# sanowl/CUDA-NT-Xent-MPI-NCCL-SimCLR

Hardware: AMD Instinct MI355X
Metric: NT-Xent fwd+bwd samples/sec, B=4096 d=2048, at 1/2/4/8 MI355X (higher is better)
Workload: dtype bf16

## Files before the change

cuda-nt-xent-mpi-nccl-simclr_amd/csrc/include/ntxent/ntxent.h:

```cpp
#pragma once

#include <hip/hip_runtime.h>

#include <cstdint>
#include <stdexcept>
#include <string>
#include <vector>

namespace ntxent {

constexpr int kWaveSize = 64;
constexpr int kTile = 256;
constexpr int kTileElems = kTile * kTile;
constexpr int kKStepBytes = 128;
constexpr int kGemmThreads = 512;
constexpr int kLdsPerCU = 160 * 1024;
constexpr int kNumXcd = 8;

enum class DType : int { F32 = 0, F16 = 1, BF16 = 2, FP8 = 3 };

inline size_t dtype_size(DType t) { return t == DType::F32 ? 4 : (t == DType::FP8 ? 1 : 2); }
inline const char* dtype_name(DType t) {
  return t == DType::F32 ? "fp32" : (t == DType::F16 ? "fp16" : (t == DType::BF16 ? "bf16" : "fp8"));
}
// ... 120 lines not shown
int q8_ldt(const Geometry& g);
struct Q8Stats {
  float* mneg2 = nullptr;
  float* lmin = nullptr;
  void* zq8t = nullptr;
  const void* zq = nullptr;
};
void launch_lse(const float2* part, const float* ypos, float* lse2_all, float* cpos,
                float* block_loss, float* loss_sum, const Geometry& g, hipStream_t stream,
                DType tr_dtype = DType::F16, const void* zq = nullptr, void* zqt = nullptr,
                const Q8Stats* q8 = nullptr, const RawRows* raw = nullptr);

int dot_slots(const Geometry& g);
void launch_coef(DType comp, const void* sbuf, void* cbuf, const float* lse2_all, const float* cpos,
                 const int4* tiles, int ntiles, const Geometry& g, hipStream_t stream,
                 void* mbuf = nullptr, float* dotp = nullptr, const Q8Stats* q8 = nullptr, bool half_c = false);
void launch_dot_reduce(const float* dotp, float* dot, const Geometry& g, hipStream_t stream);

void launch_coef_gemm(DType comp, const void* zq_local, const void* zq_all, void* cbuf,
                      const float* lse2_all, const float* cpos, const int4* tiles, int ntiles,
                      const GemmWorkspace& ws, const Geometry& g, hipStream_t stream,
                      const BlockView& bv = BlockView{}, float* dotp = nullptr);

struct NormFuse {
  const void* h = nullptr;
  DType in = DType::BF16;
  const float* inv = nullptr;
  const float* dot = nullptr;
  const float* grad_out = nullptr;
  void* dh = nullptr;
  const float* dotp = nullptr;
  int* dot_cnt = nullptr;
};
bool launch_dz(DType comp, const void* cbuf, const void* zqt_all, const int4* tiles, int ntiles,
               void* dz, const GemmWorkspace& ws, const Geometry& g, hipStream_t stream, bool out_f16 = false,
               const NormFuse* nf = nullptr, const Q8Stats* q8 = nullptr, const float* cpos = nullptr,
               bool half_c = false);
bool dz_half_c_eligible(DType comp, const Geometry& g, int n_dz, const GemmWorkspace& ws);
void set_half_c(bool on);
bool half_c_enabled();
bool dz_dot_fold_eligible(DType comp, const Geometry& g, int n_dz, const GemmWorkspace& ws);
void set_dot_fold(bool on);
bool dot_fold_enabled();
void set_dot_fold_spin(int polls);
int dot_fold_spin();

void launch_dz_view(DType comp, const void* a, long long a_panel_tiles, const void* b, long long b_kblk_cols,
                    long long b_kblk_stride, int k_tiles, const int4* tiles, int ntiles, void* out, bool accum,
                    const GemmWorkspace& ws, const Geometry& g, hipStream_t stream, bool out_f16 = false);

void launch_norm_bwd(DType in, const float* slabs, int nslabs, const void* h,
                     const float* inv, const float* grad_out, void* dh, const Geometry& g,
                     hipStream_t stream, const void* xslabs = nullptr, int nx = 0);

constexpr int kSmallMaxRows = 2048;
// ... 29 lines not shown
```

cuda-nt-xent-mpi-nccl-simclr_amd/csrc/include/ntxent/step.h:

```cpp
#pragma once

#include <hip/hip_runtime.h>

#include <cstddef>

#include "ntxent/ntxent.h"

namespace ntxent {

struct StepOverrides {
  int small_path = -1;
  int small_splits = -1;
  int fp8_backward = -1;
};

struct StepPlan {
  Geometry g;
  DType in = DType::BF16;
  DType comp = DType::F16;
  DType bwd = DType::F16;
  bool keep_cos = true;
  bool small = false;
  bool small_fwd_fused = false;
  int small_splits = 0;
  bool f8 = false;
  bool q8 = false;
  bool raw = false;
  bool fuse = false;
  bool half_c = false;
  bool dfold = false;
  int n_fwd = 0, n_own = 0, n_dz = 0;
  int num_cus = 256;
  DType fwd_mfma = DType::F16;
  DType bwd_mfma = DType::F16;
};

StepPlan resolve_step_plan(const Geometry& g, DType in, DType comp, bool keep_cos, int num_cus,
                           const StepOverrides& ov = StepOverrides{});

struct StepBuffers {
  const void* h = nullptr;
  void* zq = nullptr;
  void* zq8 = nullptr;
  void* zqt = nullptr;
// ... 46 lines not shown
```

cuda-nt-xent-mpi-nccl-simclr_amd/csrc/kernels/ntxent_kernels.hip:

```cpp

#include "../include/ntxent/ntxent.h"
#include "device_common.h"
#include "sim_gemm.h"

#include <atomic>
#include <algorithm>
#include <cmath>
#include <cstdio>
#include <cstdlib>
#include <mutex>
#include <string>
#include <type_traits>
#include <vector>
#include <unordered_map>

namespace ntxent {
namespace dev {

template <typename T> __device__ __forceinline__ void load8(const T* p, float (&v)[8]);
template <> __device__ __forceinline__ void load8<float>(const float* p, float (&v)[8]) {
  const f32x4 a = *reinterpret_cast<const f32x4*>(p), b = *reinterpret_cast<const f32x4*>(p + 4);
  v[0] = a[0]; v[1] = a[1]; v[2] = a[2]; v[3] = a[3]; v[4] = b[0]; v[5] = b[1]; v[6] = b[2]; v[7] = b[3];
}
template <typename T> __device__ __forceinline__ void load8_h(const T* p, float (&v)[8]) {
// ... 743 lines not shown
      std::fclose(fp);
    }
  }
};
#endif

template <typename Tc, int MODE>
void launch_sim_gemm(int grid, const dev::SimParams& p_in, hipStream_t stream) {
#if NTXENT_TIMING
  static TimingBuf tb;
  dev::SimParams p = p_in;
  p.tstamp = tb.prepare(grid, stream);
#else
  const dev::SimParams& p = p_in;
#endif
  if (MODE == dev::kModeFwd && !p.fixed_shift)
    hipLaunchKernelGGL((dev::sim_gemm_kernel<Tc, MODE, MODE == dev::kModeFwd ? 0 : 1>), dim3(grid), dim3(kGemmThreads), 0,
                       stream, p);
  else
    hipLaunchKernelGGL((dev::sim_gemm_kernel<Tc, MODE>), dim3(grid), dim3(kGemmThreads), 0, stream, p);
#if NTXENT_TIMING
  tb.dump("gemm_m" + std::to_string(MODE) + "_e" + std::to_string(sizeof(Tc)), grid, stream);
#endif
}

dev::SimParams base_params(const Geometry& g) {
  dev::SimParams p{};
  p.R = g.rows;
  p.Rpad = g.rows_pad;
  p.n_half = g.rows / 2;
// ... 341 lines not shown
static std::atomic<bool> g_lse_fold{[] {
  const char* e = std::getenv("NTXENT_LSE_FOLD");
  return e == nullptr || std::string(e) != "0";
}()};
void set_lse_fold(bool on) { g_lse_fold = on; }

bool lse_fold_enabled() { return g_lse_fold.load(); }
static double lse_loss_fx(const Geometry& g, int nb);

static std::atomic<bool> g_half_c{[] {
  const char* e = std::getenv("NTXENT_HALF_C");
  return e == nullptr || std::string(e) != "0";
}()};
void set_half_c(bool on) { g_half_c = on; }
bool half_c_enabled() { return g_half_c.load(); }

bool dz_half_c_eligible(DType comp, const Geometry& g, int n_dz, const GemmWorkspace& ws) {
  if ((comp != DType::F16 && comp != DType::BF16) || g.world != 1 || n_dz <= 0) return false;
  if ((long long)g.row_tiles * g.col_tiles * kTileElems * 2 >= (1ll << 31)) return false;
  const int cus = ws.sched_cus > 0 ? std::min(ws.sched_cus, ws.num_cus) : ws.num_cus;
  const int nk = (int)((long long)g.rows_pad * 2 / kKStepBytes);
  int pieces = fwd_splitk_pieces(n_dz, nk, cus, 1);
  if (pieces < 3) pieces = 0;
  if (pieces > 0) return ((nk + pieces - 1) / pieces) % 2 == 0;
  return make_schedule(n_dz, nk, cus).sk_tiles == 0;
}
static std::atomic<bool> g_dot_fold{[] {
  const char* e = std::getenv("NTXENT_DOT_FOLD");
  return e == nullptr || std::string(e) != "0";
}()};
// ... 268 lines not shown
                       static_cast<const _Float16*>(zq), q8->zq8t, g.dim_k, g.ld_k, q8_ldt(g), tx);
  } else {
    NTXENT_CHECK(zqt != nullptr, "lse: transpose output missing");
    const int tx = g.rows_pad / 64, ty = g.dim_n / 64;
    dispatch_comp(tr_dtype, [&](auto tc) {
      using Tc = decltype(tc);
      hipLaunchKernelGGL((dev::lse_transpose_kernel<Tc>), dim3(nb + tx * ty), dim3(256), 0, stream, a, nb,
                         static_cast<const Tc*>(zq), zqt, g.dim_k, g.ld_k, g.ld_t, tx);
    });
  }
  NTXENT_HIP_CHECK(hipGetLastError());
}

void launch_coef(DType comp, const void* sbuf, void* cbuf, const float* lse2_all, const float* cpos,
                 const int4* tiles, int ntiles, const Geometry& g, hipStream_t stream,
                 void* mbuf, float* dotp, const Q8Stats* q8, bool half_c) {
  if (ntiles == 0) return;
  dev::SimParams p = base_params(g);
  NTXENT_CHECK(!half_c || (mbuf == nullptr && q8 == nullptr && g.world == 1 && (comp == DType::F16 || comp == DType::BF16)),
               "coef: half C needs a 16-bit, single-rank, mirrored-layout pass");
  p.c_half = half_c ? 1 : 0;
  p.dotp = dotp;
  p.tiles = tiles;
  p.sc = const_cast<char*>(static_cast<const char*>(sbuf));
  p.cbuf = static_cast<char*>(cbuf);
  p.mbuf = static_cast<char*>(mbuf);
  if (mbuf != nullptr) {
    p.c_ld = sym_c_ld(g);
    p.c_rot = 1;
  }
  p.lse2 = lse2_all;
  p.cpos = cpos;
  if (q8) {
    NTXENT_CHECK(comp == DType::F16 && mbuf == nullptr && g.world == 1,
                 "coef (fp8 backward): fp16 kept cosines, world 1, mirrored layout");
    p.q8_mneg = q8->mneg2;
// ... 22 lines not shown
  p.nh = nf->h;
  p.nh_dt = nf->in == DType::F32 ? 0 : (nf->in == DType::F16 ? 1 : 2);
  p.nd = g.dim;
  p.ninv = nf->inv;
  p.ndot = nf->dot;
  p.ngo = nf->grad_out;
  p.nalpha = (float)(1.0 / ((double)g.global_rows * g.temperature));
  p.ndh = nf->dh;
  p.out_f16 = 1;
  p.accum = 0;
  return true;
}

bool launch_dz(DType comp, const void* sc, const void* zqt_all, const int4* tiles, int ntiles,
               void* slabs, const GemmWorkspace& ws, const Geometry& g, hipStream_t stream, bool out_f16,
               const NormFuse* nf, const Q8Stats* q8, const float* cpos, bool half_c) {
  if (ntiles == 0) return false;
  NTXENT_CHECK(!half_c || dz_half_c_eligible(comp, g, ntiles, ws), "dz: half C not eligible for this launch");
  const bool f8 = comp == DType::FP8;
  NTXENT_CHECK(!f8 || (q8 && q8->mneg2 && q8->lmin && q8->zq && cpos && g.world == 1 && out_f16),
               "dz (fp8 backward): Q8Stats, cpos, world 1 and an fp16 slab required");
  const long long cs = (long long)dtype_size(comp);
  dev::SimParams p = base_params(g);
  if (f8) {
    p.q8_mneg = q8->mneg2;
    p.q8_lmin = q8->lmin;
    p.q8_zq = static_cast<const _Float16*>(q8->zq);
    p.q8_ldz = g.ld_k;
    p.cpos = cpos;
  }
  p.A = coef_tile_operand(sc, g.col_tiles, cs);
// ... 21 lines not shown
    p.ipb = (nk + pieces - 1) / pieces;
    p.sk_cnt = static_cast<int*>(ws.ptr);
    p.sk_slabs = reinterpret_cast<float*>(static_cast<char*>(ws.ptr) + sk_counter_bytes(ws.num_cus));
    p.splitk = 1;
    grid = (int)((nk + p.ipb - 1) / p.ipb) * ntiles;
    NTXENT_CHECK(p.kbytes % kKStepBytes == 0 && grid <= ws.num_cus && ws.ptr != nullptr &&
                     ws.bytes >= gemm_workspace_bytes(ntiles, ws.num_cus),
                 "split-K dZ: workspace too small");
  } else {
    grid = apply_schedule(p, ntiles, ws, stream);
  }
  if (half_c)
    NTXENT_CHECK(((pieces == 0 && p.sk_tiles == 0 && p.dp_tiles == ntiles) || (pieces > 0 && p.ipb % 2 == 0)) &&
                     (long long)g.row_tiles * g.col_tiles * kTileElems * cs < (1ll << 31),
                 "dz: half C needs items starting at even K-steps and a C buffer below 2 GiB (32-bit offsets)");
  p.c_half = half_c ? 1 : 0;
  const bool fused = comp != DType::F32 && apply_norm_fuse(p, nf, g);
  if (fused) NTXENT_CHECK(nf->dot != nullptr, "dz: fused normalisation backward without dot");
  if (nf && nf->dot_cnt) {
    NTXENT_CHECK(fused && !f8 && nf->dotp && dz_dot_fold_eligible(comp, g, ntiles, ws),
                 "dz: dot fold needs the fused 16-bit epilogue");
    p.dotp = const_cast<float*>(nf->dotp);
    p.dot_nslot = dot_slots(g);
    p.dot_cnt = pieces == 0 ? nf->dot_cnt : nullptr;
    p.dot_spin = dot_fold_spin();
  }
  dispatch_gemm(comp, [&](auto tc) {
    using Tc = decltype(tc);
    launch_sim_gemm<Tc, dev::kModeDz>(grid, p, stream);
  });
  if (pieces > 0) hipLaunchKernelGGL(dev::sk_dz_reduce_kernel, dim3(ntiles * 64), dim3(256), 0, stream, p);
// ... 93 lines not shown
```

cuda-nt-xent-mpi-nccl-simclr_amd/csrc/kernels/sim_gemm.h:

```cpp
#pragma once

#include "../include/ntxent/ntxent.h"
#include "device_common.h"

#include <type_traits>

namespace ntxent {
namespace dev {

enum SimMode : int { kModeFwd = 0, kModeCoef = 1, kModeDz = 2 };

constexpr int kStageBytes = 2 * kTile * kKStepBytes;
#ifndef NTXENT_GEMM_DMA_AUX
#define NTXENT_GEMM_DMA_AUX 0
#endif
constexpr int kGemmDmaAux = NTXENT_GEMM_DMA_AUX;
#ifndef NTXENT_TIMING
#define NTXENT_TIMING 0
#endif
constexpr int kTimingItems = 8;
constexpr int kTimingMarks = 8;
__device__ __forceinline__ void store16_wt(void* base, long long off, u32x4 v) {
  const unsigned lo = __builtin_amdgcn_readfirstlane((unsigned)off);
  const unsigned hi = __builtin_amdgcn_readfirstlane((unsigned)((unsigned long long)off >> 32));
// ... 82 lines not shown
  __device__ __forceinline__ void init(const char* base, long long k0, const OperandDesc& o, int nk) {
    kin = (int)(k0 % o.kblk);
    ptr = base + (k0 / o.kblk) * o.kblk_stride + kin;
    left = nk - 1;
    kk = (int)(k0 / kKStepBytes);
  }
  __device__ __forceinline__ void advance(const OperandDesc& o) {
    if (left > 0) {
      --left;
      ++kk;
      ptr += kKStepBytes;
      kin += kKStepBytes;
      if (kin == (int)o.kblk) { kin = 0; ptr += o.kblk_stride - o.kblk; }
    }
  }
  __device__ __forceinline__ void skip() {
    if (left > 0) {
      --left;
      ++kk;
    }
  }
  __device__ __forceinline__ void seek(const char* base, long long k0, const OperandDesc& o) {
    kin = (int)(k0 % o.kblk);
    ptr = base + (k0 / o.kblk) * o.kblk_stride + kin;
  }
};

__device__ __forceinline__ int ct_swz(int L) {
  return ((L >> 1) & 1) | ((L & 1) << 1) | (((L >> 3) & 1) << 2) | ((((L >> 1) ^ (L >> 2)) & 1) << 3);
}

__device__ __forceinline__ void dot_slot_store(float* p, float v) { *p = v; }

__device__ __forceinline__ long long ctile_index(const SimParams& p, int mt, int nt) {
  const int cs = p.c_rot ? (nt - p.row_tile0 + p.col_tiles) % p.col_tiles : nt - p.c_tile0;
  return (long long)mt * p.c_ld + cs;
}

template <typename T, int NW, int NMI = 8>
__device__ __forceinline__ void coef_epilogue(f32x4 (&acc)[NMI][4], const int (&rb)[NMI], const int (&cb)[4],
// ... 14 lines not shown
  const bool fixed = p.fixed_shift != 0;
  const float M = p.y_scale;
  float lcol[4];
  bool cvalid[4];
  int gj[4];
#pragma unroll
  for (int ni = 0; ni < 4; ++ni) {
    const int col_t = cb[ni] + (lane & 15);
    gj[ni] = nt * kTile + col_t;
    const float l = p.lse2[gj[ni]];
    lcol[ni] = fixed ? fast_exp2(M - l) : l;
    cvalid[ni] = (col_local0 + col_t) < p.R;
  }
  T* slot = base + ctile_index(p, mt, nt) * kTileElems;
  T* mirror = nullptr;
  if ((kind == kTileSymOff && !p.c_half) || kind == kTileDiagUp)
    mirror = base + ctile_index(p, nt - p.row_tile0, p.row_tile0 + mt) * kTileElems;
  else if (kind == kTileCross) {
    const int rt = p.Rpad / kTile, W = p.col_tiles / rt, q = nt / rt;
    const int slot = (q - p.row_tile0 / rt - 1 + W) % W;
    mirror = reinterpret_cast<T*>(p.mbuf) + ((long long)(slot * rt + nt % rt) * rt + mt) * kTileElems;
  }
  const int wq = NW == 8 ? ((threadIdx.x >> 6) & 3) : (col_base >> 6);
  float cdot[2][4] = {{0.f, 0.f, 0.f, 0.f}, {0.f, 0.f, 0.f, 0.f}};
  const int r_lo = mt * kTile + row_base, r_hi = r_lo + NROWS;
  const int c_lo = nt * kTile + col_base, c_hi = c_lo + NCOLS;
  auto hits = [&](int a0) { return a0 < c_hi && c_lo < a0 + NROWS; };
  const bool plain = fixed && r_hi <= p.R && col_local0 + col_base + NCOLS <= p.R && !hits(p.own0 + r_lo) &&
                     !hits(p.own0 + r_lo + p.n_half) && !hits(p.own0 + r_lo - p.n_half);
#pragma unroll
  for (int mi = 0; mi < NMI; ++mi) {
// ... 87 lines not shown
        u32x4 v;
        if constexpr (SWZ) {
          typedef __attribute__((address_space(3))) const u32x2 lds_u2;
          const u32x2 lo = *(lds_u2*)(lds + ct_at(row, 8 * c16)), hi = *(lds_u2*)(lds + ct_at(row, 8 * c16 + 4));
          v = u32x4{lo[0], lo[1], hi[0], hi[1]};
        } else {
          v = *reinterpret_cast<const __attribute__((address_space(3))) u32x4*>(lds + row * S + c16 * 16);
        }
        *reinterpret_cast<u32x4*>(reinterpret_cast<char*>(mirror) + ctile_off(col_base + row, row_base + 8 * c16, 2)) = v;
      }
    }
    typedef short v4s __attribute__((ext_vector_type(4)));
    constexpr int RB = NROWS / 16;
    constexpr int NBLK = RB * (NCOLS / 32) / NW;
    const int g = lane >> 4, i = lane & 15, q4 = i >> 2, p4 = i & 3;
#pragma unroll 2
    for (int b = 0; b < NBLK; ++b) {
      const int blk = w * NBLK + b;
      const int c0 = (blk % RB) * 16;
      const int r0 = (blk / RB) * 32 + 8 * g;
      const lds_char* a0 = lds + ct_at(r0 + q4, c0 + 4 * p4);
      const lds_char* a1 = lds + ct_at(r0 + q4 + 4, c0 + 4 * p4);
      const v4s lo = __builtin_amdgcn_ds_read_tr16_b64_v4i16((__attribute__((address_space(3))) v4s*)a0);
      const v4s hi = __builtin_amdgcn_ds_read_tr16_b64_v4i16((__attribute__((address_space(3))) v4s*)a1);
      u32x4 u;
      u[0] = (unsigned short)lo[0] | ((unsigned)(unsigned short)lo[1] << 16);
      u[1] = (unsigned short)lo[2] | ((unsigned)(unsigned short)lo[3] << 16);
      u[2] = (unsigned short)hi[0] | ((unsigned)(unsigned short)hi[1] << 16);
      u[3] = (unsigned short)hi[2] | ((unsigned)(unsigned short)hi[3] << 16);
      const int src = ((lane >> 2) + 16 * (lane & 3)) << 2;
// ... 558 lines not shown
  const int wa = w >> 2, wb = w & 3;
  const int G = gridDim.x;
  const int bid = xcd_remap(blockIdx.x, G);
  const int nk = p.nk;
  KStream sa0, sa1, sb0, sb1;

  unsigned a_vo[2], b_vo[2];
#pragma unroll
  for (int j = 0; j < 2; ++j) {
    const int rl = 8 * j + (lane >> 3);
    const int lchunk = (lane & 7) ^ ((rl >> 1) & 7);
    a_vo[j] = (unsigned)((lane >> 3) * p.A.ld) + lchunk * 16;
    b_vo[j] = (unsigned)((lane >> 3) * p.B.ld) + lchunk * 16;
  }
  constexpr bool kTrCap = MODE == kModeDz && sizeof(T) == 2 && !std::is_same<T, fp8e4m3>::value;
  int tr_end = 0;
  const char* tr_base = nullptr;
  unsigned a_tr_vo = 0, rd_tr = 0;
  if constexpr (kTrCap) {
    const int x = w & 1;
    const int ch = 8 * (((lane >> 3) & 1) ^ x) + 2 * (lane >> 4) + (lane & 1);
    a_tr_vo = (unsigned)(((lane >> 1) & 3) * p.A.ld + 16 * ch);
    const int g = lane >> 4, q = (lane >> 2) & 3, pp = lane & 3;
    rd_tr = (unsigned)(2048 * g + 128 * (wa ^ (g & 1)) + 32 * q + 16 * (pp >> 1) + 8 * (pp & 1));
    asm volatile("" : "+v"(a_tr_vo), "+v"(rd_tr));
  }
  auto stage = [&](int isB, int h, KStream& s, int buf, int trm = 1) {
    lds_char* dst = lds + isB * kStageBytes + buf * (kTile * kKStepBytes) + (128 * h + 16 * w) * kKStepBytes;
    if constexpr (kTrCap) {
      if (!isB && (trm == 2 || (trm == 1 && s.kk < tr_end))) {
        const unsigned so = (unsigned)(s.kk >> 2) * (unsigned)p.A.row_tile_stride +
                            (unsigned)(((s.kk & 3) * 64 + 8 * w) * (int)p.A.ld + 256 * h);
        const auto trs = __builtin_amdgcn_make_buffer_rsrc(const_cast<char*>(tr_base), 0, 0x7FFFFFFF, 0x00020000);
#pragma unroll
        for (int j = 0; j < 2; ++j)
          __builtin_amdgcn_raw_ptr_buffer_load_lds(trs, (lds_void*)(dst + 8 * j * kKStepBytes), 16, a_tr_vo,
                                                   so + (unsigned)(4 * j * (int)p.A.ld), 0, kGemmDmaAux);
        s.skip();
        return;
      }
    }
    const auto rs = __builtin_amdgcn_make_buffer_rsrc(const_cast<char*>(s.ptr), 0, 0x7FFFFFFF, 0x00020000);
#pragma unroll
    for (int j = 0; j < 2; ++j)
      __builtin_amdgcn_raw_ptr_buffer_load_lds(rs, (lds_void*)(dst + 8 * j * kKStepBytes), 16, isB ? b_vo[j] : a_vo[j],
                                               (unsigned)((128 * h + 16 * w + 8 * j) * (isB ? p.B.ld : p.A.ld)), 0,
                                               kGemmDmaAux);
    s.advance(isB ? p.B : p.A);
  };
  auto stage_h = [&](int i, int mt_, int nt_) {
    const long long hld = (long long)p.nd * 2;
    const char* hb = static_cast<const char*>(p.nh) + ((long long)mt_ * kTile + 128 * (i & 1)) * hld +
                     (long long)nt_ * kTile * 2 + 128 * (i >> 1);
// ... 153 lines not shown
      return true;
    }
    if (it >= it1) return false;
    stile = (int)(it / nk);
    kb = (int)(it % nk);
    ke = (int)((long long)kb + (it1 - it) < nk ? kb + (it1 - it) : nk);
    it += ke - kb;
    tile = p.dp_tiles + stile;
    return true;
  };
  auto prologue = [&](int tile, int kb, int ke, int slot) {
    const int4 tt = sload_int4(p.tiles, tile);
    if (p.inv_a) stage_inv(tt.x, tt.y, slot);
    if constexpr (kTrCap) {
      tr_base = p.A.base + (long long)tt.x * p.A.kblk_stride;
      tr_end = p.c_half ? 4 * tt.x : 0;
    }
    const int ns = ke - kb;
    const char* Ab = p.A.base + (long long)tt.x * p.A.row_tile_stride;
    const char* Bb = p.B.base + (long long)(tt.y - p.b_tile0) * p.B.row_tile_stride;
    const long long k0 = (long long)kb * kKStepBytes;
    sa0.init(Ab, k0, p.A, ns); sa1.init(Ab, k0, p.A, ns);
    if constexpr (kTrCap) {
      if (tr_end > kb) {
        sa0.seek(Ab, (long long)tr_end * kKStepBytes, p.A);
        sa1.seek(Ab, (long long)tr_end * kKStepBytes, p.A);
      }
    }
    sb0.init(Bb, k0, p.B, ns); sb1.init(Bb, k0, p.B, ns);
    if constexpr (kF8 && MODE != kModeDz) {
      const int t = threadIdx.x;
      const char* src = (t < 256 ? Ab + (long long)t * p.A.ld : Bb + (long long)(t - 256) * p.B.ld) + p.scale_off;
      __builtin_amdgcn_global_load_lds((const void*)src, (lds_void*)(lds + kScaleLds + 256 * w), 4, 0, 0);
    }
    stage(0, 0, sa0, 0); stage(1, 0, sb0, 0); stage(1, 1, sb1, 0); stage(0, 1, sa1, 0);
    stage(0, 0, sa0, 1); stage(1, 0, sb0, 1); stage(1, 1, sb1, 1);
  };
  const bool streaming = kStreamMode && p.sk_tiles == 0 && nk >= 2 && (nk & 1) == 0;
  bool streamed = false;
  int dstate = 0;
  bool dot_counted = false;
  if constexpr (MODE == kModeDz && !kF8 && sizeof(T) == 2) {
    if (p.dot_nslot > 0) dz_dot_fold(p, lds + kGemmLds, threadIdx.x);
// ... 42 lines not shown
  if constexpr (kF8 && MODE != kModeDz) {
    const int r16_ = lane & 15;
    unsigned av[8], bv[4];
    lds_get_scales((unsigned)(uintptr_t)(lds + kScaleLds) + 4 * (64 * wa + r16_),
                   (unsigned)(uintptr_t)(lds + kScaleLds) + 4 * (256 + 32 * wb + r16_), av, bv);
    sa_v[0] = pack_low_bytes(av[0], av[1], av[2], av[3]);
    sa_v[1] = pack_low_bytes(av[4], av[5], av[6], av[7]);
    sb_v = pack_low_bytes(bv[0], bv[1], bv[2], bv[3]);
  }
  tmark(item, 1);
  if (grp == 1) barrier();
  bool hpre = false;
  if constexpr (MODE == kModeDz && !kF8)
    hpre = p.ndh != nullptr && (p.nh_dt == 1 || p.nh_dt == 2) && stile < 0 && nsteps == nk && nsteps >= 4 &&
           (nsteps & 1) == 0 && p.R % kTile == 0 && p.nd % kTile == 0;
  auto kstep = [&](const int ks, auto cur_c, auto tail_c, auto tr_c) {
    constexpr int cur = decltype(cur_c)::value, nxt = cur ^ 1;
    constexpr int TAIL = decltype(tail_c)::value;
    constexpr bool TR = decltype(tr_c)::value != 0;
    constexpr int TRM = decltype(tr_c)::value == 0 ? 0 : (decltype(tr_c)::value == 2 ? 1 : 2);
    if constexpr (kStreamMode) {
      if (cont && ks == nsteps - 2) {
        sa0.init(na, 0, p.A, nk); sb0.init(nb, 0, p.B, nk); sb1.init(nb, 0, p.B, nk);
        if (p.inv_a) stage_inv(nmt, nnt, (item + 1) & 1);
      }
      if (cont && ks == nsteps - 1) sa1.init(na, 0, p.A, nk);
    }
    dma_wait(); barrier();
    if constexpr (TR) read_a_tr(cur_c, kI0, af);
    else read_a(cur, 0, af);
    __builtin_amdgcn_sched_barrier(0);
    read_b(cur, 0, bf0);
    if constexpr (TAIL == 2) stage_h(3, mt, nt);
    else stage(0, 1, sa1, nxt, TRM);
    a0_retire(); barrier();
    lds_drain();
    if constexpr (TR) __builtin_amdgcn_sched_barrier(0);
    mma_quadrant(kI0, kI0, af, bf0);
    dma_wait(); barrier();
    read_b(cur, 1, bf1);
    if constexpr (TAIL != 0) stage_h(TAIL == 1 ? 0 : 4, mt, nt);
    else stage(0, 0, sa0, cur, TRM);
    barrier(); lds_drain();
    mma_quadrant(kI0, kI1, af, bf1);
    barrier();
    if constexpr (TR) read_a_tr(cur_c, kI1, af);
    else read_a(cur, 1, af);
    if constexpr (TAIL != 0) stage_h(TAIL == 1 ? 1 : 5, mt, nt);
    else stage(1, 0, sb0, cur);
    barrier(); lds_drain();
    if constexpr (TR) __builtin_amdgcn_sched_barrier(0);
    mma_quadrant(kI1, kI0, af, bf0);
    if constexpr (TAIL != 2) dma_wait();
    barrier();
    if constexpr (TAIL != 0) {
      stage_h(TAIL == 1 ? 2 : 6, mt, nt);
      if constexpr (TAIL == 2) stage_h(7, mt, nt);
    } else {
      stage(1, 1, sb1, cur);
    }
    barrier();
    mma_quadrant(kI1, kI1, af, bf1);
  };
  const std::integral_constant<int, 2> kI2{};
  int ks2 = 0;
  const int nmain = nsteps - (hpre ? 2 : 0);
  if constexpr (kTrCap) {
    const int ntr = tr_end > kb ? (tr_end < ke ? tr_end : ke) - kb : 0;
    for (; ks2 + 3 < ntr; ks2 += 2) {
      kstep(ks2, kI0, kI0, kI1);
      kstep(ks2 + 1, kI1, kI0, kI1);
    }
    if (ks2 + 1 < ntr) {
      kstep(ks2, kI0, kI0, kI2);
      kstep(ks2 + 1, kI1, kI0, kI2);
      ks2 += 2;
    }
  }
  for (; ks2 + 1 < nmain; ks2 += 2) {
    kstep(ks2, kI0, kI0, kI0);
    kstep(ks2 + 1, kI1, kI0, kI0);
  }
  if constexpr (MODE == kModeDz && !kF8) {
    if (hpre) {
      kstep(ks2, kI0, kI1, kI0);
      kstep(ks2 + 1, kI1, kI2, kI0);
      ks2 += 2;
    }
  }
  if (ks2 < nsteps) kstep(ks2, kI0, kI0, kI0);
  if (grp == 0) barrier();
  tmark(item, 2);
  float hiv = 0.f, hdt = 0.f;
  if constexpr (MODE == kModeDz && !kF8) {
    if (hpre && threadIdx.x < kTile) {
      hiv = p.ninv[mt * kTile + threadIdx.x];
      hdt = dz_dot<sizeof(T) == 2>(p, mt * kTile + threadIdx.x, dstate);
    }
  }
  if (kStreamMode && cont) {
    streamed = true;
  } else {
    streamed = false;
    asm volatile("s_waitcnt vmcnt(0)" ::: "memory");
  }
// ... 891 lines not shown
```

cuda-nt-xent-mpi-nccl-simclr_amd/csrc/runtime/ntxent_torch.cpp:

```cpp
#include <torch/extension.h>
#include <ATen/hip/impl/HIPGuardImplMasqueradingAsCUDA.h>
#include <ATen/hip/impl/HIPStreamMasqueradingAsCUDA.h>
#include <ATen/hip/impl/HIPCachingAllocatorMasqueradingAsCUDA.h>

#include <algorithm>
#include <map>
#include <memory>
#include <atomic>
#include <mutex>
#include <string>
#include <tuple>
#include <vector>

#include "ntxent/engine.h"
#include "ntxent/ntxent.h"
#include "ntxent/step.h"

namespace ntxent {
namespace th {

DType to_dtype(at::ScalarType t) {
  switch (t) {
    case at::kFloat: return DType::F32;
    case at::kHalf: return DType::F16;
    case at::kBFloat16: return DType::BF16;
    default: NTXENT_CHECK(false, std::string("unsupported dtype ") + c10::toString(t));
  }
  return DType::F32;
}
// ... 892 lines not shown
  m.def("fwd_stats", [](const at::Tensor& zl, const at::Tensor& za, const Plan& P, bool keep) {
    return fwd_stats(zl, za, P, keep, true);
  }, py::arg("zq_local"), py::arg("zq_all"), py::arg("plan"), py::arg("keep_cos"));
  m.def("lse", &lse, py::arg("part"), py::arg("ypos"), py::arg("lse2_all"), py::arg("cpos"), py::arg("plan"),
        py::arg("zq") = py::none(), py::arg("zqt") = py::none());
  m.def("coef", &coef, py::arg("sbuf"), py::arg("lse2_all"), py::arg("cpos"), py::arg("plan"));
  m.def("coef_gemm", &coef_gemm);
  m.def("dz", &dz);
  m.def("set_fp8_backward", &ntxent::set_fp8_backward, py::arg("on"));
  m.def("set_raw_forward", &ntxent::set_raw_forward, py::arg("on"));
  m.def("raw_forward_enabled", &ntxent::raw_forward_enabled);
  m.def("set_lse_fold", &ntxent::set_lse_fold, py::arg("on"));
  m.def("lse_fold_enabled", &ntxent::lse_fold_enabled);
  m.def("set_half_c", &ntxent::set_half_c, py::arg("on"));
  m.def("half_c_enabled", &ntxent::half_c_enabled);
  m.def("set_dot_fold", &ntxent::set_dot_fold, py::arg("on"));
  m.def("dot_fold_enabled", &ntxent::dot_fold_enabled);
  m.def("set_dot_fold_spin", &ntxent::set_dot_fold_spin, py::arg("polls"));
  m.def("dot_fold_spin", &ntxent::dot_fold_spin);
  m.def("fp8_backward_enabled", &ntxent::fp8_backward_enabled);
  m.def("fwd_splitk_pieces", &ntxent::fwd_splitk_pieces, py::arg("ntiles"), py::arg("nk"), py::arg("cus"),
        py::arg("diag_tail"));
  m.def("fwd_diag_remainder", &ntxent::fwd_diag_remainder, py::arg("ntiles"), py::arg("nk"), py::arg("cus"),
        py::arg("diag_tail"), py::arg("f8") = false);
  m.def("norm_bwd", &norm_bwd, py::arg("slabs"), py::arg("h"), py::arg("inv"), py::arg("grad_out"), py::arg("plan"));
  m.def("fwd_stats_tiles", &fwd_stats_tiles, py::arg("zq_local"), py::arg("zq_chunk"), py::arg("b_tile0"),
        py::arg("tiles"), py::arg("plan"), py::arg("part"), py::arg("reserve_cus") = 0);
  m.def("coef_gemm_tiles", &coef_gemm_tiles, py::arg("zq_local"), py::arg("zq_chunk"), py::arg("b_tile0"),
        py::arg("tiles"), py::arg("lse2_all"), py::arg("cpos"), py::arg("plan"), py::arg("c_ld"), py::arg("c_tile0"),
        py::arg("reserve_cus") = 0);
// ... 63 lines not shown
    const auto s = ntxent::make_schedule(ntiles, nk, num_cus);
    py::dict r;
    r["grid"] = s.grid; r["nk"] = s.nk; r["dp_tiles"] = s.dp_tiles; r["sk_tiles"] = s.sk_tiles;
    r["ipb"] = s.ipb;
    return r;
  }, py::arg("ntiles"), py::arg("nk"), py::arg("num_cus"));
  m.def("gemm_workspace_bytes", &ntxent::gemm_workspace_bytes);
  m.def("step_plan", [](int rows, int dim, const std::string& input, const std::string& compute, bool keep_cos,
                        int num_cus) {
    const ntxent::DType comp = parse_dtype_name(compute);
    const auto p = ntxent::resolve_step_plan(ntxent::make_geometry(rows, dim, 1, 0, 0.07f), parse_dtype_name(input),
                                             comp, keep_cos || comp == ntxent::DType::FP8, num_cus);
    py::dict r;
    r["small"] = p.small; r["small_fwd_fused"] = p.small_fwd_fused; r["small_splits"] = p.small_splits;
    r["f8"] = p.f8; r["q8"] = p.q8; r["raw"] = p.raw; r["fuse"] = p.fuse; r["half_c"] = p.half_c;
    r["dfold"] = p.dfold; r["keep_cos"] = p.keep_cos; r["bwd"] = ntxent::dtype_name(p.bwd);
    r["n_fwd"] = p.n_fwd; r["n_own"] = p.n_own; r["n_dz"] = p.n_dz;
    r["forward_mfma"] = ntxent::dtype_name(p.fwd_mfma); r["backward_mfma"] = ntxent::dtype_name(p.bwd_mfma);
    return r;
  }, py::arg("rows"), py::arg("dim"), py::arg("input"), py::arg("compute"), py::arg("keep_cos") = true,
     py::arg("num_cus") = 256);
  m.attr("TILE") = ntxent::kTile;
  m.attr("K_STEP_BYTES") = ntxent::kKStepBytes;
}
```

cuda-nt-xent-mpi-nccl-simclr_amd/csrc/runtime/step.cpp:

```cpp
#include "ntxent/step.h"

#include <algorithm>

#include "ntxent/trace.h"

namespace ntxent {

StepPlan resolve_step_plan(const Geometry& g, DType in, DType comp, bool keep_cos, int num_cus,
                           const StepOverrides& ov) {
  StepPlan p;
  p.g = g;
  p.in = in;
  p.comp = comp;
  p.bwd = backward_dtype(comp);
  p.keep_cos = keep_cos;
  p.num_cus = num_cus;
  p.f8 = comp == DType::FP8;
  p.n_own = count_own_fwd_tiles(g);
  p.n_fwd = p.n_own + g.row_tiles * (g.col_tiles - g.row_tiles);
  p.n_dz = g.row_tiles * (g.dim_n / kTile);
  p.fwd_mfma = comp;
  p.bwd_mfma = p.bwd;
  p.small = (ov.small_path < 0 ? small_path_enabled() : ov.small_path != 0) && small_path_eligible(g, comp);
  if (p.small) {
    p.small_fwd_fused = small_fwd_fused(g);
    const int o = ov.small_splits < 0 ? small_splits_override() : ov.small_splits;
    p.small_splits = o > 0 ? std::min(o, small_rows_pad(g) / 64) : small_bwd_splits(g);
    return p;
  }
  p.q8 = keep_cos && fp8_backward_eligible(g, comp) &&
         (ov.fp8_backward < 0 ? fp8_backward_enabled() : ov.fp8_backward != 0);
  p.raw = keep_cos && !p.f8 && raw_forward_enabled() && raw_forward_eligible(g, in, comp);
  p.fuse = !p.f8 && p.bwd != DType::F32 && g.dim % 8 == 0;
  GemmWorkspace ws;
  ws.num_cus = num_cus;
  p.half_c = keep_cos && !p.q8 && half_c_enabled() && dz_half_c_eligible(p.bwd, g, p.n_dz, ws);
  p.dfold = p.fuse && !p.q8 && dz_dot_fold_eligible(p.bwd, g, p.n_dz, ws);
  p.fwd_mfma = p.raw ? in : comp;
  p.bwd_mfma = p.q8 ? DType::FP8 : p.bwd;
  return p;
}

StepBufferBytes step_buffer_bytes(const StepPlan& p) {
  const Geometry& g = p.g;
  const size_t W = g.world, Rp = g.rows_pad, R = g.rows, cs = dtype_size(p.bwd);
  StepBufferBytes n;
  n.zq = W * Rp * g.ld_k * cs;
  n.inv = n.ypos = R * 4;
  if (p.small) {
    n.lse2 = n.cpos = (size_t)small_rows_pad(g) * 4;
    n.small_scratch = small_scratch_bytes(g, std::max(small_bwd_splits(g), p.small_splits));
// ... 107 lines not shown
    launch_small_bwd(p.in, p.comp, b.zq, b.h, b.inv, b.lse2, b.cpos, b.grad_out, b.dh, b.small_scratch, g, s,
                     p.small_splits);
    return;
  }
  const char* zq_local = slot(b.zq, (size_t)g.rows_pad * g.ld_k * dtype_size(p.bwd), g);
  Q8Stats q8;
  q8.mneg2 = b.q8_mneg;
  q8.lmin = b.q8_lmin;
  q8.zq = zq_local;
  float* dotp = p.fuse ? b.dotp : nullptr;
  {
    NTXENT_TRACE("ntxent.coef");
    fault_point("coef");
    if (p.keep_cos)
      launch_coef(p.bwd, b.sbuf, b.cbuf, b.lse2, b.cpos, b.fwd_tiles, p.n_fwd, g, s, nullptr, dotp,
                  p.q8 ? &q8 : nullptr, p.half_c);
    else
      launch_coef_gemm(p.bwd, zq_local, b.zq, b.cbuf, b.lse2, b.cpos, b.fwd_tiles, p.n_fwd, b.ws, g, s, BlockView{},
                       dotp);
    if (p.fuse && !p.dfold) launch_dot_reduce(b.dotp, b.dot, g, s);
  }
  if (comm) comm->before_dz(s);
  {
    NTXENT_TRACE("ntxent.dz_gemm");
    fault_point("dz");
    NormFuse nf;
    nf.h = b.h;
    nf.in = p.in;
    nf.inv = b.inv;
    nf.dot = b.dot;
    nf.grad_out = b.grad_out;
    nf.dh = b.dh;
    if (p.dfold) {
      nf.dotp = b.dotp;
      nf.dot_cnt = b.dot_cnt;
    }
    const bool fused =
        p.q8 ? launch_dz(DType::FP8, b.cbuf, b.zq8t, b.dz_tiles, p.n_dz, b.slabs, b.ws, g, s, true,
                         p.fuse ? &nf : nullptr, &q8, b.cpos)
             : launch_dz(p.bwd, b.cbuf, b.zqt, b.dz_tiles, p.n_dz, b.slabs, b.ws, g, s,
                         p.bwd != DType::F32, p.fuse ? &nf : nullptr, nullptr, nullptr, p.half_c);
    if (fused) return;
  }
  {
    NTXENT_TRACE("ntxent.norm_bwd");
    fault_point("norm_bwd");
    if (p.bwd != DType::F32)
      launch_norm_bwd(p.in, nullptr, 0, b.h, b.inv, b.grad_out, b.dh, g, s, b.slabs, 1);
    else
      launch_norm_bwd(p.in, static_cast<const float*>(b.slabs), 1, b.h, b.inv, b.grad_out, b.dh, g, s);
  }
}

}
```

Measured before the change: 10.34 million.

## Balance half-C symmetric tile storage with a circular split to even out dz work

With half-C on, each symmetric off-diagonal tile pair is now stored by a circular-distance rule instead of the upper triangle, so each row tile owns about half of its partners. In the dz GEMM, transposed reads of the C panel become one wraparound run per row tile, and the K loop is split into up to four alternating normal and transposed segments chosen at runtime. The aim is to stop row tiles near the end of the triangle from doing all their K-steps through the slower transposed path, which leaves the load uneven across workgroups. The cost is extra scalar control flow, runtime-selected transpose staging at segment boundaries, and a new K-step limit check. It is on by default behind an environment variable, but only for single-rank runs.

```diff
diff --git a/cuda-nt-xent-mpi-nccl-simclr_amd/csrc/include/ntxent/half_c.h b/cuda-nt-xent-mpi-nccl-simclr_amd/csrc/include/ntxent/half_c.h
--- /dev/null
+++ b/cuda-nt-xent-mpi-nccl-simclr_amd/csrc/include/ntxent/half_c.h
@@ -0,0 +1,20 @@
+#pragma once
+
+namespace ntxent {
+
+constexpr bool half_c_stored(int I, int J, int T, bool balance) {
+  if (!balance) return J >= I;
+  const int d = J >= I ? J - I : J - I + T;
+  return 2 * d < T || (2 * d == T && 2 * I < T);
+}
+
+struct HalfCRun {
+  int start, len;
+};
+constexpr HalfCRun half_c_tr_run(int I, int T, bool balance) {
+  if (!balance) return HalfCRun{0, I};
+  const int dmin = (T % 2 != 0 || 2 * I < T) ? T / 2 + 1 : T / 2;
+  return HalfCRun{(I + dmin) % T, T - dmin};
+}
+
+}
diff --git a/cuda-nt-xent-mpi-nccl-simclr_amd/csrc/include/ntxent/ntxent.h b/cuda-nt-xent-mpi-nccl-simclr_amd/csrc/include/ntxent/ntxent.h
--- a/cuda-nt-xent-mpi-nccl-simclr_amd/csrc/include/ntxent/ntxent.h
+++ b/cuda-nt-xent-mpi-nccl-simclr_amd/csrc/include/ntxent/ntxent.h
@@ -158,7 +158,8 @@
 int dot_slots(const Geometry& g);
 void launch_coef(DType comp, const void* sbuf, void* cbuf, const float* lse2_all, const float* cpos,
                  const int4* tiles, int ntiles, const Geometry& g, hipStream_t stream,
-                 void* mbuf = nullptr, float* dotp = nullptr, const Q8Stats* q8 = nullptr, bool half_c = false);
+                 void* mbuf = nullptr, float* dotp = nullptr, const Q8Stats* q8 = nullptr, bool half_c = false,
+                 bool half_c_balance = false);
 void launch_dot_reduce(const float* dotp, float* dot, const Geometry& g, hipStream_t stream);
 
 void launch_coef_gemm(DType comp, const void* zq_local, const void* zq_all, void* cbuf,
@@ -179,10 +180,12 @@
 bool launch_dz(DType comp, const void* cbuf, const void* zqt_all, const int4* tiles, int ntiles,
                void* dz, const GemmWorkspace& ws, const Geometry& g, hipStream_t stream, bool out_f16 = false,
                const NormFuse* nf = nullptr, const Q8Stats* q8 = nullptr, const float* cpos = nullptr,
-               bool half_c = false);
+               bool half_c = false, bool half_c_balance = false);
 bool dz_half_c_eligible(DType comp, const Geometry& g, int n_dz, const GemmWorkspace& ws);
 void set_half_c(bool on);
 bool half_c_enabled();
+void set_half_c_balance(bool on);
+bool half_c_balance_enabled();
 bool dz_dot_fold_eligible(DType comp, const Geometry& g, int n_dz, const GemmWorkspace& ws);
 void set_dot_fold(bool on);
 bool dot_fold_enabled();
diff --git a/cuda-nt-xent-mpi-nccl-simclr_amd/csrc/include/ntxent/step.h b/cuda-nt-xent-mpi-nccl-simclr_amd/csrc/include/ntxent/step.h
--- a/cuda-nt-xent-mpi-nccl-simclr_amd/csrc/include/ntxent/step.h
+++ b/cuda-nt-xent-mpi-nccl-simclr_amd/csrc/include/ntxent/step.h
@@ -28,6 +28,7 @@
   bool raw = false;
   bool fuse = false;
   bool half_c = false;
+  bool half_c_balance = false;
   bool dfold = false;
   int n_fwd = 0, n_own = 0, n_dz = 0;
   int num_cus = 256;
diff --git a/cuda-nt-xent-mpi-nccl-simclr_amd/csrc/kernels/ntxent_kernels.hip b/cuda-nt-xent-mpi-nccl-simclr_amd/csrc/kernels/ntxent_kernels.hip
--- a/cuda-nt-xent-mpi-nccl-simclr_amd/csrc/kernels/ntxent_kernels.hip
+++ b/cuda-nt-xent-mpi-nccl-simclr_amd/csrc/kernels/ntxent_kernels.hip
@@ -1,4 +1,5 @@
 
+#include "../include/ntxent/half_c.h"
 #include "../include/ntxent/ntxent.h"
 #include "device_common.h"
 #include "sim_gemm.h"
@@ -781,6 +782,7 @@
 #else
   const dev::SimParams& p = p_in;
 #endif
+  NTXENT_CHECK(p.nk < (1 << 16), "similarity GEMM: more than 65535 K-steps per tile");
   if (MODE == dev::kModeFwd && !p.fixed_shift)
     hipLaunchKernelGGL((dev::sim_gemm_kernel<Tc, MODE, MODE == dev::kModeFwd ? 0 : 1>), dim3(grid), dim3(kGemmThreads), 0,
                        stream, p);
@@ -1152,6 +1154,12 @@
 }()};
 void set_half_c(bool on) { g_half_c = on; }
 bool half_c_enabled() { return g_half_c.load(); }
+static std::atomic<bool> g_half_c_balance{[] {
+  const char* e = std::getenv("NTXENT_HALF_C_BALANCE");
+  return e == nullptr || std::string(e) != "0";
+}()};
+void set_half_c_balance(bool on) { g_half_c_balance = on; }
+bool half_c_balance_enabled() { return g_half_c_balance.load(); }
 
 bool dz_half_c_eligible(DType comp, const Geometry& g, int n_dz, const GemmWorkspace& ws) {
   if ((comp != DType::F16 && comp != DType::BF16) || g.world != 1 || n_dz <= 0) return false;
@@ -1450,12 +1458,12 @@
 
 void launch_coef(DType comp, const void* sbuf, void* cbuf, const float* lse2_all, const float* cpos,
                  const int4* tiles, int ntiles, const Geometry& g, hipStream_t stream,
-                 void* mbuf, float* dotp, const Q8Stats* q8, bool half_c) {
+                 void* mbuf, float* dotp, const Q8Stats* q8, bool half_c, bool half_c_balance) {
   if (ntiles == 0) return;
   dev::SimParams p = base_params(g);
   NTXENT_CHECK(!half_c || (mbuf == nullptr && q8 == nullptr && g.world == 1 && (comp == DType::F16 || comp == DType::BF16)),
                "coef: half C needs a 16-bit, single-rank, mirrored-layout pass");
-  p.c_half = half_c ? 1 : 0;
+  p.c_half = half_c ? (half_c_balance ? 2 : 1) : 0;
   p.dotp = dotp;
   p.tiles = tiles;
   p.sc = const_cast<char*>(static_cast<const char*>(sbuf));
@@ -1508,7 +1516,7 @@
 
 bool launch_dz(DType comp, const void* sc, const void* zqt_all, const int4* tiles, int ntiles,
                void* slabs, const GemmWorkspace& ws, const Geometry& g, hipStream_t stream, bool out_f16,
-               const NormFuse* nf, const Q8Stats* q8, const float* cpos, bool half_c) {
+               const NormFuse* nf, const Q8Stats* q8, const float* cpos, bool half_c, bool half_c_balance) {
   if (ntiles == 0) return false;
   NTXENT_CHECK(!half_c || dz_half_c_eligible(comp, g, ntiles, ws), "dz: half C not eligible for this launch");
   const bool f8 = comp == DType::FP8;
@@ -1560,7 +1568,7 @@
     NTXENT_CHECK(((pieces == 0 && p.sk_tiles == 0 && p.dp_tiles == ntiles) || (pieces > 0 && p.ipb % 2 == 0)) &&
                      (long long)g.row_tiles * g.col_tiles * kTileElems * cs < (1ll << 31),
                  "dz: half C needs items starting at even K-steps and a C buffer below 2 GiB (32-bit offsets)");
-  p.c_half = half_c ? 1 : 0;
+  p.c_half = half_c ? (half_c_balance ? 2 : 1) : 0;
   const bool fused = comp != DType::F32 && apply_norm_fuse(p, nf, g);
   if (fused) NTXENT_CHECK(nf->dot != nullptr, "dz: fused normalisation backward without dot");
   if (nf && nf->dot_cnt) {
diff --git a/cuda-nt-xent-mpi-nccl-simclr_amd/csrc/kernels/sim_gemm.h b/cuda-nt-xent-mpi-nccl-simclr_amd/csrc/kernels/sim_gemm.h
--- a/cuda-nt-xent-mpi-nccl-simclr_amd/csrc/kernels/sim_gemm.h
+++ b/cuda-nt-xent-mpi-nccl-simclr_amd/csrc/kernels/sim_gemm.h
@@ -1,5 +1,6 @@
 #pragma once
 
+#include "../include/ntxent/half_c.h"
 #include "../include/ntxent/ntxent.h"
 #include "device_common.h"
 
@@ -120,16 +121,6 @@
       if (kin == (int)o.kblk) { kin = 0; ptr += o.kblk_stride - o.kblk; }
     }
   }
-  __device__ __forceinline__ void skip() {
-    if (left > 0) {
-      --left;
-      ++kk;
-    }
-  }
-  __device__ __forceinline__ void seek(const char* base, long long k0, const OperandDesc& o) {
-    kin = (int)(k0 % o.kblk);
-    ptr = base + (k0 / o.kblk) * o.kblk_stride + kin;
-  }
 };
 
 __device__ __forceinline__ int ct_swz(int L) {
@@ -174,7 +165,9 @@
   }
   T* slot = base + ctile_index(p, mt, nt) * kTileElems;
   T* mirror = nullptr;
-  if ((kind == kTileSymOff && !p.c_half) || kind == kTileDiagUp)
+  const bool half_off = kind == kTileSymOff && p.c_half != 0;
+  const bool direct = !half_off || half_c_stored(mt, nt, p.col_tiles, p.c_half == 2);
+  if ((kind == kTileSymOff && (!half_off || !direct)) || kind == kTileDiagUp)
     mirror = base + ctile_index(p, nt - p.row_tile0, p.row_tile0 + mt) * kTileElems;
   else if (kind == kTileCross) {
     const int rt = p.Rpad / kTile, W = p.col_tiles / rt, q = nt / rt;
@@ -292,6 +285,7 @@
     constexpr int RB = NROWS / 16;
     constexpr int NBLK = RB * (NCOLS / 32) / NW;
     const int g = lane >> 4, i = lane & 15, q4 = i >> 2, p4 = i & 3;
+    if (direct)
 #pragma unroll 2
     for (int b = 0; b < NBLK; ++b) {
       const int blk = w * NBLK + b;
@@ -880,8 +874,12 @@
     b_vo[j] = (unsigned)((lane >> 3) * p.B.ld) + lchunk * 16;
   }
   constexpr bool kTrCap = MODE == kModeDz && sizeof(T) == 2 && !std::is_same<T, fp8e4m3>::value;
-  int tr_end = 0;
+  int tr_s = 0, tr_len = 0;
   const char* tr_base = nullptr;
+  auto is_tr = [&](int kk) {
+    const int u = kk - tr_s;
+    return (u < 0 ? u + nk : u) < tr_len;
+  };
   unsigned a_tr_vo = 0, rd_tr = 0;
   if constexpr (kTrCap) {
     const int x = w & 1;
@@ -894,7 +892,7 @@
   auto stage = [&](int isB, int h, KStream& s, int buf, int trm = 1) {
     lds_char* dst = lds + isB * kStageBytes + buf * (kTile * kKStepBytes) + (128 * h + 16 * w) * kKStepBytes;
     if constexpr (kTrCap) {
-      if (!isB && (trm == 2 || (trm == 1 && s.kk < tr_end))) {
+      if (!isB && (trm == 2 || (trm == 1 && is_tr(s.kk)))) {
         const unsigned so = (unsigned)(s.kk >> 2) * (unsigned)p.A.row_tile_stride +
                             (unsigned)(((s.kk & 3) * 64 + 8 * w) * (int)p.A.ld + 256 * h);
         const auto trs = __builtin_amdgcn_make_buffer_rsrc(const_cast<char*>(tr_base), 0, 0x7FFFFFFF, 0x00020000);
@@ -902,7 +900,7 @@
         for (int j = 0; j < 2; ++j)
           __builtin_amdgcn_raw_ptr_buffer_load_lds(trs, (lds_void*)(dst + 8 * j * kKStepBytes), 16, a_tr_vo,
                                                    so + (unsigned)(4 * j * (int)p.A.ld), 0, kGemmDmaAux);
-        s.skip();
+        s.advance(p.A);
         return;
       }
     }
@@ -1086,19 +1084,15 @@
     if (p.inv_a) stage_inv(tt.x, tt.y, slot);
     if constexpr (kTrCap) {
       tr_base = p.A.base + (long long)tt.x * p.A.kblk_stride;
-      tr_end = p.c_half ? 4 * tt.x : 0;
+      const HalfCRun run = half_c_tr_run(tt.x, p.col_tiles, p.c_half == 2);
+      tr_s = 4 * run.start;
+      tr_len = p.c_half ? 4 * run.len : 0;
     }
     const int ns = ke - kb;
     const char* Ab = p.A.base + (long long)tt.x * p.A.row_tile_stride;
     const char* Bb = p.B.base + (long long)(tt.y - p.b_tile0) * p.B.row_tile_stride;
     const long long k0 = (long long)kb * kKStepBytes;
     sa0.init(Ab, k0, p.A, ns); sa1.init(Ab, k0, p.A, ns);
-    if constexpr (kTrCap) {
-      if (tr_end > kb) {
-        sa0.seek(Ab, (long long)tr_end * kKStepBytes, p.A);
-        sa1.seek(Ab, (long long)tr_end * kKStepBytes, p.A);
-      }
-    }
     sb0.init(Bb, k0, p.B, ns); sb1.init(Bb, k0, p.B, ns);
     if constexpr (kF8 && MODE != kModeDz) {
       const int t = threadIdx.x;
@@ -1171,11 +1165,21 @@
   if constexpr (MODE == kModeDz && !kF8)
     hpre = p.ndh != nullptr && (p.nh_dt == 1 || p.nh_dt == 2) && stile < 0 && nsteps == nk && nsteps >= 4 &&
            (nsteps & 1) == 0 && p.R % kTile == 0 && p.nd % kTile == 0;
-  auto kstep = [&](const int ks, auto cur_c, auto tail_c, auto tr_c) {
+  auto kstep = [&](const int ks, auto cur_c, auto tail_c, auto tr_c, auto s1_c, auto s2_c) {
     constexpr int cur = decltype(cur_c)::value, nxt = cur ^ 1;
     constexpr int TAIL = decltype(tail_c)::value;
-    constexpr bool TR = decltype(tr_c)::value != 0;
-    constexpr int TRM = decltype(tr_c)::value == 0 ? 0 : (decltype(tr_c)::value == 2 ? 1 : 2);
+    constexpr bool kRt = std::is_same<decltype(tr_c), bool>::value;
+    bool TR;
+    int TRM1, TRM2;
+    if constexpr (kRt) {
+      TR = tr_c; TRM1 = s1_c ? 2 : 0; TRM2 = s2_c ? 2 : 0;
+    } else {
+      TR = decltype(tr_c)::value != 0; TRM1 = 2 * decltype(s1_c)::value; TRM2 = 2 * decltype(s2_c)::value;
+    }
+    auto tr_pin = [&]() {
+      if constexpr (kRt) __builtin_amdgcn_sched_barrier(0);
+      else if constexpr (decltype(tr_c)::value != 0) __builtin_amdgcn_sched_barrier(0);
+    };
     if constexpr (kStreamMode) {
       if (cont && ks == nsteps - 2) {
         sa0.init(na, 0, p.A, nk); sb0.init(nb, 0, p.B, nk); sb1.init(nb, 0, p.B, nk);
@@ -1184,29 +1188,29 @@
       if (cont && ks == nsteps - 1) sa1.init(na, 0, p.A, nk);
     }
     dma_wait(); barrier();
-    if constexpr (TR) read_a_tr(cur_c, kI0, af);
+    if (kTrCap && TR) read_a_tr(cur_c, kI0, af);
     else read_a(cur, 0, af);
     __builtin_amdgcn_sched_barrier(0);
     read_b(cur, 0, bf0);
     if constexpr (TAIL == 2) stage_h(3, mt, nt);
-    else stage(0, 1, sa1, nxt, TRM);
+    else stage(0, 1, sa1, nxt, TRM1);
     a0_retire(); barrier();
     lds_drain();
-    if constexpr (TR) __builtin_amdgcn_sched_barrier(0);
+    tr_pin();
     mma_quadrant(kI0, kI0, af, bf0);
     dma_wait(); barrier();
     read_b(cur, 1, bf1);
     if constexpr (TAIL != 0) stage_h(TAIL == 1 ? 0 : 4, mt, nt);
-    else stage(0, 0, sa0, cur, TRM);
+    else stage(0, 0, sa0, cur, TRM2);
     barrier(); lds_drain();
     mma_quadrant(kI0, kI1, af, bf1);
     barrier();
-    if constexpr (TR) read_a_tr(cur_c, kI1, af);
+    if (kTrCap && TR) read_a_tr(cur_c, kI1, af);
     else read_a(cur, 1, af);
     if constexpr (TAIL != 0) stage_h(TAIL == 1 ? 1 : 5, mt, nt);
     else stage(1, 0, sb0, cur);
     barrier(); lds_drain();
-    if constexpr (TR) __builtin_amdgcn_sched_barrier(0);
+    tr_pin();
     mma_quadrant(kI1, kI0, af, bf0);
     if constexpr (TAIL != 2) dma_wait();
     barrier();
@@ -1222,30 +1226,58 @@
   const std::integral_constant<int, 2> kI2{};
   int ks2 = 0;
   const int nmain = nsteps - (hpre ? 2 : 0);
+  bool tr_tail = false;
+  if constexpr (kTrCap) tr_tail = hpre && is_tr(ke - 2);
+  auto kpair = [&](const int ks, auto cm_c, auto sm_c) {
+    kstep(ks, kI0, kI0, cm_c, cm_c, sm_c);
+    kstep(ks + 1, kI1, kI0, cm_c, sm_c, sm_c);
+  };
   if constexpr (kTrCap) {
-    const int ntr = tr_end > kb ? (tr_end < ke ? tr_end : ke) - kb : 0;
-    for (; ks2 + 3 < ntr; ks2 += 2) {
-      kstep(ks2, kI0, kI0, kI1);
-      kstep(ks2 + 1, kI1, kI0, kI1);
-    }
-    if (ks2 + 1 < ntr) {
-      kstep(ks2, kI0, kI0, kI2);
-      kstep(ks2 + 1, kI1, kI0, kI2);
-      ks2 += 2;
-    }
-  }
-  for (; ks2 + 1 < nmain; ks2 += 2) {
-    kstep(ks2, kI0, kI0, kI0);
-    kstep(ks2 + 1, kI1, kI0, kI0);
+    unsigned e01, e23;
+    {
+      int pos = 0, e[4];
+#pragma unroll
+      for (int i = 0; i < 4; ++i) {
+        if (pos < nsteps) {
+          const int k = kb + pos;
+          int u = k - tr_s;
+          u = u < 0 ? u + nk : u;
+          const bool cm = u < tr_len;
+          if (cm == ((i & 1) == 0)) {
+            const int re = k - u + (cm ? tr_len : nk);
+            pos = (re < ke ? re : ke) - kb;
+          }
+        }
+        e[i] = pos;
+      }
+      e01 = (unsigned)e[0] | ((unsigned)e[1] << 16);
+      e23 = (unsigned)e[2] | ((unsigned)e[3] << 16);
+      asm volatile("" : "+s"(e01), "+s"(e23));
+    }
+    auto seg = [&](const int re, auto cm_c, auto om_c) {
+      const int lim = re < nmain ? re : nmain;
+      const int same = re < nsteps ? re - 2 : lim;
+      for (; ks2 + 1 < same; ks2 += 2) kpair(ks2, cm_c, cm_c);
+      if (ks2 + 1 < lim) {
+        kpair(ks2, cm_c, om_c);
+        ks2 += 2;
+      }
+    };
+    seg((int)(e01 & 0xffffu), kI1, kI0);
+    seg((int)(e01 >> 16), kI0, kI1);
+    seg((int)(e23 & 0xffffu), kI1, kI0);
+    seg((int)(e23 >> 16), kI0, kI1);
+  } else {
+    for (; ks2 + 1 < nmain; ks2 += 2) kpair(ks2, kI0, kI0);
   }
   if constexpr (MODE == kModeDz && !kF8) {
     if (hpre) {
-      kstep(ks2, kI0, kI1, kI0);
-      kstep(ks2 + 1, kI1, kI2, kI0);
+      kstep(ks2, kI0, kI1, tr_tail, tr_tail, tr_tail);
+      kstep(ks2 + 1, kI1, kI2, tr_tail, tr_tail, tr_tail);
       ks2 += 2;
     }
   }
-  if (ks2 < nsteps) kstep(ks2, kI0, kI0, kI0);
+  if (ks2 < nsteps) kstep(ks2, kI0, kI0, kI0, kI0, kI0);
   if (grp == 0) barrier();
   tmark(item, 2);
   float hiv = 0.f, hdt = 0.f;
diff --git a/cuda-nt-xent-mpi-nccl-simclr_amd/csrc/runtime/ntxent_torch.cpp b/cuda-nt-xent-mpi-nccl-simclr_amd/csrc/runtime/ntxent_torch.cpp
--- a/cuda-nt-xent-mpi-nccl-simclr_amd/csrc/runtime/ntxent_torch.cpp
+++ b/cuda-nt-xent-mpi-nccl-simclr_amd/csrc/runtime/ntxent_torch.cpp
@@ -13,6 +13,7 @@
 #include <vector>
 
 #include "ntxent/engine.h"
+#include "ntxent/half_c.h"
 #include "ntxent/ntxent.h"
 #include "ntxent/step.h"
 
@@ -935,6 +936,15 @@
   m.def("lse_fold_enabled", &ntxent::lse_fold_enabled);
   m.def("set_half_c", &ntxent::set_half_c, py::arg("on"));
   m.def("half_c_enabled", &ntxent::half_c_enabled);
+  m.def("set_half_c_balance", &ntxent::set_half_c_balance, py::arg("on"));
+  m.def("half_c_balance_enabled", &ntxent::half_c_balance_enabled);
+  m.def("half_c_stored", [](int I, int J, int T, py::object balance) {
+    return ntxent::half_c_stored(I, J, T, balance.is_none() ? ntxent::half_c_balance_enabled() : balance.cast<bool>());
+  }, py::arg("I"), py::arg("J"), py::arg("T"), py::arg("balance") = py::none());
+  m.def("half_c_tr_run", [](int I, int T, py::object balance) {
+    const auto r = ntxent::half_c_tr_run(I, T, balance.is_none() ? ntxent::half_c_balance_enabled() : balance.cast<bool>());
+    return py::make_tuple(r.start, r.len);
+  }, py::arg("I"), py::arg("T"), py::arg("balance") = py::none());
   m.def("set_dot_fold", &ntxent::set_dot_fold, py::arg("on"));
   m.def("dot_fold_enabled", &ntxent::dot_fold_enabled);
   m.def("set_dot_fold_spin", &ntxent::set_dot_fold_spin, py::arg("polls"));
@@ -1028,6 +1038,7 @@
     py::dict r;
     r["small"] = p.small; r["small_fwd_fused"] = p.small_fwd_fused; r["small_splits"] = p.small_splits;
     r["f8"] = p.f8; r["q8"] = p.q8; r["raw"] = p.raw; r["fuse"] = p.fuse; r["half_c"] = p.half_c;
+    r["half_c_balance"] = p.half_c_balance;
     r["dfold"] = p.dfold; r["keep_cos"] = p.keep_cos; r["bwd"] = ntxent::dtype_name(p.bwd);
     r["n_fwd"] = p.n_fwd; r["n_own"] = p.n_own; r["n_dz"] = p.n_dz;
     r["forward_mfma"] = ntxent::dtype_name(p.fwd_mfma); r["backward_mfma"] = ntxent::dtype_name(p.bwd_mfma);
diff --git a/cuda-nt-xent-mpi-nccl-simclr_amd/csrc/runtime/step.cpp b/cuda-nt-xent-mpi-nccl-simclr_amd/csrc/runtime/step.cpp
--- a/cuda-nt-xent-mpi-nccl-simclr_amd/csrc/runtime/step.cpp
+++ b/cuda-nt-xent-mpi-nccl-simclr_amd/csrc/runtime/step.cpp
@@ -35,6 +35,7 @@
   GemmWorkspace ws;
   ws.num_cus = num_cus;
   p.half_c = keep_cos && !p.q8 && half_c_enabled() && dz_half_c_eligible(p.bwd, g, p.n_dz, ws);
+  p.half_c_balance = p.half_c && half_c_balance_enabled();
   p.dfold = p.fuse && !p.q8 && dz_dot_fold_eligible(p.bwd, g, p.n_dz, ws);
   p.fwd_mfma = p.raw ? in : comp;
   p.bwd_mfma = p.q8 ? DType::FP8 : p.bwd;
@@ -172,7 +173,7 @@
     fault_point("coef");
     if (p.keep_cos)
       launch_coef(p.bwd, b.sbuf, b.cbuf, b.lse2, b.cpos, b.fwd_tiles, p.n_fwd, g, s, nullptr, dotp,
-                  p.q8 ? &q8 : nullptr, p.half_c);
+                  p.q8 ? &q8 : nullptr, p.half_c, p.half_c_balance);
     else
       launch_coef_gemm(p.bwd, zq_local, b.zq, b.cbuf, b.lse2, b.cpos, b.fwd_tiles, p.n_fwd, b.ws, g, s, BlockView{},
                        dotp);
@@ -197,7 +198,8 @@
         p.q8 ? launch_dz(DType::FP8, b.cbuf, b.zq8t, b.dz_tiles, p.n_dz, b.slabs, b.ws, g, s, true,
                          p.fuse ? &nf : nullptr, &q8, b.cpos)
              : launch_dz(p.bwd, b.cbuf, b.zqt, b.dz_tiles, p.n_dz, b.slabs, b.ws, g, s,
-                         p.bwd != DType::F32, p.fuse ? &nf : nullptr, nullptr, nullptr, p.half_c);
+                         p.bwd != DType::F32, p.fuse ? &nf : nullptr, nullptr, nullptr, p.half_c,
+                         p.half_c_balance);
     if (fused) return;
   }
   {
```

Result: no change. 10.32 million (-0.2%).
